# DeonDavisV/Nodexa-Chain-Core

Hardware: AMD Instinct MI355X
Metric: KawPow MH/s + Equihash(200,9) Sol/s, whole node at 1/2/4/8 MI355X (higher is better)
Workload: dtype u32; 1 GPU; model=KawPow (ProgPoW 0.9.4, RAVENCOINKAWPOW) epoch 384, 4.00 GiB DAG, height 2880123, global_batch=33553920, parallelism=dp1

## Files before the change

nodexa_chain_core_amd/hip/kernels/kawpow_anyperiod.hip:

```cpp
#include "kernel_params.h"
#include "keccak_device.hpp"

#define KA_BLOCK 256
#define KA_MIN_WAVES 6

NX_DEV uint32_t ka_fnv1a(uint32_t h, uint32_t d) { return (h ^ d) * 0x01000193u; }
NX_DEV uint32_t ka_mod(uint32_t x, const FastMod32& f) {
    const uint32_t r = x - __umulhi(x, f.mb) * f.d;
    return min(r, r - f.d);
}
NX_DEV uint32_t ka_clz(uint32_t x) { return x ? (uint32_t)__builtin_clz(x) : 32u; }

NX_DEV uint32_t ka_merge(uint32_t a, uint32_t b, uint32_t kind, uint32_t rot) {
    switch (kind) {
        case 0: return a * 33u + b;
        case 1: return (a ^ b) * 33u;
        case 2: return __builtin_rotateleft32(a, rot) ^ b;
        default: return __builtin_rotateright32(a, rot) ^ b;
    }
}

NX_DEV uint32_t ka_math(uint32_t a, uint32_t b, uint32_t kind) {
    switch (kind) {
        case 0: return a + b;
        case 1: return a * b;
        case 2: return __umulhi(a, b);
        case 3: return min(a, b);
        case 4: return __builtin_rotateleft32(a, b);
        case 5: return __builtin_rotateright32(a, b);
        case 6: return a & b;
        case 7: return a | b;
        case 8: return a ^ b;
        case 9: return ka_clz(a) + ka_clz(b);
        default: return (uint32_t)(__builtin_popcount(a) + __builtin_popcount(b));
    }
}

typedef uint32_t ka_mix_t __attribute__((ext_vector_type(32)));
NX_DEV uint32_t ka_get(const ka_mix_t& m, uint32_t i) { return m[i & 31]; }
NX_DEV void ka_set(ka_mix_t& m, uint32_t i, uint32_t v) { m[i & 31] = v; }

NX_DEV void ka_seed(const uint32_t header[8], uint64_t nonce, uint32_t st2[8]) {
    uint32_t s[25];
#pragma unroll
    for (int i = 0; i < 8; ++i) s[i] = header[i];
    s[8] = (uint32_t)nonce;
    s[9] = (uint32_t)(nonce >> 32);
    const uint32_t pad[15] = {0x72, 0x41, 0x56, 0x45, 0x4E, 0x43, 0x4F, 0x49, 0x4E, 0x4B, 0x41, 0x57, 0x50, 0x4F, 0x57};
#pragma unroll
    for (int i = 0; i < 15; ++i) s[10 + i] = pad[i];
    keccak_f800(s);
#pragma unroll
    for (int i = 0; i < 8; ++i) st2[i] = s[i];
}

NX_DEV void ka_final(const uint32_t st2[8], const uint32_t digest[8], uint32_t out[8]) {
    uint32_t s[25];
#pragma unroll
    for (int i = 0; i < 8; ++i) s[i] = st2[i];
#pragma unroll
    for (int i = 0; i < 8; ++i) s[8 + i] = digest[i];
    const uint32_t pad[9] = {0x72, 0x41, 0x56, 0x45, 0x4E, 0x43, 0x4F, 0x49, 0x4E};
#pragma unroll
    for (int i = 0; i < 9; ++i) s[16 + i] = pad[i];
    keccak_f800(s);
#pragma unroll
    for (int i = 0; i < 8; ++i) out[i] = s[i];
}

struct KaProgram {
    uint32_t w[51];
};
NX_DEV void ka_load_program(KaProgram& pg, const uint32_t* program) {
#pragma unroll
    for (int i = 0; i < 51; ++i) pg.w[i] = __builtin_amdgcn_readfirstlane(program[i]);
}

NX_DEV void ka_group_hashes(const uint4* __restrict__ dag, const FastMod32& items, const uint32_t* l1,
                            KaProgram& pg, uint32_t st0, uint32_t st1, uint32_t lane, uint32_t (&own)[8]) {
#pragma unroll 1
    for (uint32_t h = 0; h < 16; ++h) {
        ka_mix_t mix;
        {
            const uint32_t z0 = ka_fnv1a(0x811c9dc5u, __shfl(st0, (int)h, 16));
            const uint32_t w0 = ka_fnv1a(z0, __shfl(st1, (int)h, 16));
            const uint32_t jsr0 = ka_fnv1a(w0, lane);
            uint32_t kz = z0, kw = w0, kj = jsr0, kc = ka_fnv1a(jsr0, lane);
#pragma unroll
            for (int r = 0; r < 32; ++r) {
                kz = 36969u * (kz & 0xffffu) + (kz >> 16);
                kw = 18000u * (kw & 0xffffu) + (kw >> 16);
                kc = 69069u * kc + 1234567u;
                kj ^= (kj << 17);
                kj ^= (kj >> 13);
                kj ^= (kj << 5);
                mix[r] = (((kz << 16) + kw) ^ kc) + kj;
            }
        }
#pragma unroll 1
        for (uint32_t r = 0; r < 64; ++r) {
            const uint32_t index = ka_mod(__shfl(mix[0], (int)(r & 15), 16), items);
            const uint4 d = dag[(size_t)index * 16 + ((lane ^ r) & 15)];
#pragma unroll
            for (int i = 0; i < 51; ++i) asm volatile("" : "+s"(pg.w[i]));
#pragma unroll
            for (int i = 0; i < 18; ++i) {
                if (i < 11) {
                    const uint32_t op = pg.w[i];
                    const uint32_t dst = (op >> 8) & 31;
                    ka_set(mix, dst, ka_merge(ka_get(mix, dst), l1[ka_get(mix, op) & 4095u], (op >> 16) & 3, op >> 24));
                }
                const uint32_t op = pg.w[11 + i];
                const uint32_t mg = pg.w[29 + i];
                const uint32_t dst = op >> 24;
                const uint32_t v = ka_math(ka_get(mix, op), ka_get(mix, op >> 8), (op >> 16) & 15);
                ka_set(mix, dst, ka_merge(ka_get(mix, dst), v, mg & 3, mg >> 8));
            }
            const uint32_t dw[4] = {d.x, d.y, d.z, d.w};
#pragma unroll
            for (int i = 0; i < 4; ++i) {
                const uint32_t op = pg.w[47 + i];
                ka_set(mix, op, ka_merge(ka_get(mix, op), dw[i], (op >> 8) & 3, op >> 16));
            }
        }
        uint32_t lh = 0x811c9dc5u;
#pragma unroll
        for (int r = 0; r < 32; ++r) lh = ka_fnv1a(lh, mix[r]);
        const bool mine = lane == h;
#pragma unroll
        for (int k = 0; k < 8; ++k) {
            const uint32_t a = __shfl(lh, k, 16);
            const uint32_t b = __shfl(lh, k + 8, 16);
            const uint32_t word = ka_fnv1a(ka_fnv1a(0x811c9dc5u, a), b);
            own[k] = mine ? word : own[k];
        }
    }
}

extern "C" __global__ __launch_bounds__(KA_BLOCK, KA_MIN_WAVES) void kawpow_search_any(KawpowAnySearchParams p) {
    __shared__ uint32_t l1[4096];
    __shared__ uint32_t stale_word;
    if (blockDim.x != KA_BLOCK) return;
    if (threadIdx.x == 0) {
        uint32_t s = 0;
        if (p.gen_word) s = __hip_atomic_load(p.gen_word, __ATOMIC_RELAXED, __HIP_MEMORY_SCOPE_SYSTEM) != p.generation;
        stale_word = s;
        if (s) atomicAdd(&p.results->skipped, 1u);
    }
    for (int i = threadIdx.x; i < 4096; i += KA_BLOCK) l1[i] = p.l1[i];
    __syncthreads();
    if (stale_word) return;

    KaProgram pg;
    ka_load_program(pg, p.program);
    const uint32_t lane = threadIdx.x & 15;
    const uint4* dag = (const uint4*)p.dag;
#pragma unroll 1
    for (uint32_t t = threadIdx.x; t < p.granule; t += KA_BLOCK) {
        const uint64_t nonce = p.start_nonce + (uint64_t)blockIdx.x * p.granule + t;
        uint32_t st2[8], digest[8] = {0, 0, 0, 0, 0, 0, 0, 0}, fin[8];
        ka_seed(p.header, nonce, st2);
        ka_group_hashes(dag, p.items, l1, pg, st2[0], st2[1], lane, digest);
        ka_final(st2, digest, fin);
        const uint64_t head = ((uint64_t)__builtin_bswap32(fin[0]) << 32) | __builtin_bswap32(fin[1]);
        if (head <= p.target) {
            const uint32_t slot = atomicAdd(&p.results->count, 1u);
            if (slot < NODEXA_KAWPOW_MAX_SHARES) {
                KawpowShare* s = &p.results->shares[slot];
                s->nonce = nonce;
#pragma unroll
                for (int k = 0; k < 8; ++k) {
                    s->mix[k] = digest[k];
                    s->final_[k] = fin[k];
                }
            }
        }
    }
}

extern "C" __global__ __launch_bounds__(KA_BLOCK, KA_MIN_WAVES) void kawpow_hash_any(KawpowAnyHashParams p) {
    __shared__ uint32_t l1[4096];
    if (blockDim.x != KA_BLOCK) return;
    for (int i = threadIdx.x; i < 4096; i += KA_BLOCK) l1[i] = p.l1[i];
    __syncthreads();
    KaProgram pg;
    ka_load_program(pg, p.program);
    const uint32_t lane = threadIdx.x & 15;
    const uint32_t job = blockIdx.x * KA_BLOCK + threadIdx.x;
    const bool valid = job < p.num_jobs;
    const KawpowVerifyJob j = p.jobs[valid ? job : 0];
    uint32_t st2[8], digest[8] = {0, 0, 0, 0, 0, 0, 0, 0}, fin[8];
    ka_seed(j.header, j.nonce, st2);
    ka_group_hashes((const uint4*)p.dag, p.items, l1, pg, st2[0], st2[1], lane, digest);
    ka_final(st2, digest, fin);
    if (valid) {
        uint32_t* o = p.out + (size_t)job * 16;
#pragma unroll
        for (int k = 0; k < 8; ++k) {
            o[k] = digest[k];
            o[8 + k] = fin[k];
        }
    }
}
```

Before: 292.8 MH/s.

## Interleave two ProgPoW lane-hash chains per thread and compact program words

The inner ProgPoW loop now advances KA_H (default 2) independent mix states at once, so each thread issues two DAG loads per round and interleaves their dependent ALU chains to gain instruction-level parallelism. Program words are packed from 51 to 33 SGPRs, and rotate-left merges are rewritten as rotate-right so one switch case disappears. The seed Keccak is recomputed after the loop instead of keeping st2 live, which trades extra Keccak work for fewer live registers. Occupancy drops from 6 to 4 minimum waves to make room for the doubled 32-word mix arrays, which risks spilling or less latency hiding.

```diff
diff --git a/nodexa_chain_core_amd/hip/kernels/kawpow_anyperiod.hip b/nodexa_chain_core_amd/hip/kernels/kawpow_anyperiod.hip
--- a/nodexa_chain_core_amd/hip/kernels/kawpow_anyperiod.hip
+++ b/nodexa_chain_core_amd/hip/kernels/kawpow_anyperiod.hip
@@ -2,7 +2,27 @@
 #include "keccak_device.hpp"
 
 #define KA_BLOCK 256
-#define KA_MIN_WAVES 6
+#ifndef KA_H
+#define KA_H 2
+#endif
+#ifndef KA_MIN_WAVES
+#define KA_MIN_WAVES 4
+#endif
+#ifndef KA_RESEED
+#define KA_RESEED 1
+#endif
+#ifndef KA_ROTR_ONLY
+#define KA_ROTR_ONLY 1
+#endif
+#if KA_H == 1
+#define KA_EACH(X) X(0)
+#elif KA_H == 2
+#define KA_EACH(X) X(0) X(1)
+#elif KA_H == 4
+#define KA_EACH(X) X(0) X(1) X(2) X(3)
+#else
+#error "KA_H must be 1, 2 or 4"
+#endif
 
 NX_DEV uint32_t ka_fnv1a(uint32_t h, uint32_t d) { return (h ^ d) * 0x01000193u; }
 NX_DEV uint32_t ka_mod(uint32_t x, const FastMod32& f) {
@@ -11,34 +31,35 @@
 }
 NX_DEV uint32_t ka_clz(uint32_t x) { return x ? (uint32_t)__builtin_clz(x) : 32u; }
 
-NX_DEV uint32_t ka_merge(uint32_t a, uint32_t b, uint32_t kind, uint32_t rot) {
+#define KA_FOR_H _Pragma("unroll") for (int k = 0; k < KA_H; ++k)
+NX_DEV void ka_merge(uint32_t (&a)[KA_H], const uint32_t (&b)[KA_H], uint32_t kind, uint32_t rot) {
     switch (kind) {
-        case 0: return a * 33u + b;
-        case 1: return (a ^ b) * 33u;
-        case 2: return __builtin_rotateleft32(a, rot) ^ b;
-        default: return __builtin_rotateright32(a, rot) ^ b;
-    }
-}
-
-NX_DEV uint32_t ka_math(uint32_t a, uint32_t b, uint32_t kind) {
+        case 0: KA_FOR_H a[k] = a[k] * 33u + b[k]; break;
+        case 1: KA_FOR_H a[k] = (a[k] ^ b[k]) * 33u; break;
+#if !KA_ROTR_ONLY
+        case 2: KA_FOR_H a[k] = __builtin_rotateleft32(a[k], rot) ^ b[k]; break;
+#endif
+        default: KA_FOR_H a[k] = __builtin_rotateright32(a[k], rot) ^ b[k]; break;
+    }
+}
+
+NX_DEV void ka_math(uint32_t (&v)[KA_H], const uint32_t (&a)[KA_H], const uint32_t (&b)[KA_H], uint32_t kind) {
     switch (kind) {
-        case 0: return a + b;
-        case 1: return a * b;
-        case 2: return __umulhi(a, b);
-        case 3: return min(a, b);
-        case 4: return __builtin_rotateleft32(a, b);
-        case 5: return __builtin_rotateright32(a, b);
-        case 6: return a & b;
-        case 7: return a | b;
-        case 8: return a ^ b;
-        case 9: return ka_clz(a) + ka_clz(b);
-        default: return (uint32_t)(__builtin_popcount(a) + __builtin_popcount(b));
+        case 0: KA_FOR_H v[k] = a[k] + b[k]; break;
+        case 1: KA_FOR_H v[k] = a[k] * b[k]; break;
+        case 2: KA_FOR_H v[k] = __umulhi(a[k], b[k]); break;
+        case 3: KA_FOR_H v[k] = min(a[k], b[k]); break;
+        case 4: KA_FOR_H v[k] = __builtin_rotateleft32(a[k], b[k]); break;
+        case 5: KA_FOR_H v[k] = __builtin_rotateright32(a[k], b[k]); break;
+        case 6: KA_FOR_H v[k] = a[k] & b[k]; break;
+        case 7: KA_FOR_H v[k] = a[k] | b[k]; break;
+        case 8: KA_FOR_H v[k] = a[k] ^ b[k]; break;
+        case 9: KA_FOR_H v[k] = ka_clz(a[k]) + ka_clz(b[k]); break;
+        default: KA_FOR_H v[k] = (uint32_t)(__builtin_popcount(a[k]) + __builtin_popcount(b[k])); break;
     }
 }
 
 typedef uint32_t ka_mix_t __attribute__((ext_vector_type(32)));
-NX_DEV uint32_t ka_get(const ka_mix_t& m, uint32_t i) { return m[i & 31]; }
-NX_DEV void ka_set(ka_mix_t& m, uint32_t i, uint32_t v) { m[i & 31] = v; }
 
 NX_DEV void ka_seed(const uint32_t header[8], uint64_t nonce, uint32_t st2[8]) {
     uint32_t s[25];
@@ -69,70 +90,141 @@
 }
 
 struct KaProgram {
-    uint32_t w[51];
+    uint32_t w[33];
 };
+NX_DEV void ka_rotr_only(uint32_t& kind, uint32_t& rot) {
+#if KA_ROTR_ONLY
+    if (kind == 2u) {
+        kind = 3u;
+        rot = (32u - rot) & 31u;
+    }
+#endif
+}
 NX_DEV void ka_load_program(KaProgram& pg, const uint32_t* program) {
 #pragma unroll
-    for (int i = 0; i < 51; ++i) pg.w[i] = __builtin_amdgcn_readfirstlane(program[i]);
+    for (int i = 0; i < 11; ++i) {
+        const uint32_t w = __builtin_amdgcn_readfirstlane(program[i]);
+        uint32_t kind = (w >> 16) & 3u, rot = (w >> 24) & 31u;
+        ka_rotr_only(kind, rot);
+        pg.w[i] = (w & 0xffffu) | (kind << 16) | (rot << 24);
+    }
+#pragma unroll
+    for (int i = 0; i < 18; ++i) {
+        const uint32_t op = __builtin_amdgcn_readfirstlane(program[11 + i]);
+        const uint32_t mg = __builtin_amdgcn_readfirstlane(program[29 + i]);
+        uint32_t kind = mg & 3u, rot = (mg >> 8) & 31u;
+        ka_rotr_only(kind, rot);
+        pg.w[11 + i] = (op & 31u) | (((op >> 8) & 31u) << 5) | (((op >> 16) & 15u) << 10) | (((op >> 24) & 31u) << 14) |
+                       (kind << 19) | (rot << 21);
+    }
+#pragma unroll
+    for (int i = 0; i < 4; ++i) {
+        const uint32_t w = __builtin_amdgcn_readfirstlane(program[47 + i]);
+        uint32_t kind = (w >> 8) & 3u, rot = (w >> 16) & 31u;
+        ka_rotr_only(kind, rot);
+        pg.w[29 + i] = (w & 0xffu) | (kind << 8) | (rot << 16);
+    }
+}
+
+#define KA_MIX(k) m##k
+#define KA_GET(k, dstarr, idx) dstarr[k] = KA_MIX(k)[(idx) & 31];
+#define KA_SET(k, srcarr, idx) KA_MIX(k)[(idx) & 31] = srcarr[k];
+
+NX_DEV ka_mix_t ka_fill(uint32_t s0, uint32_t s1, uint32_t lane) {
+    ka_mix_t mix;
+    const uint32_t z0 = ka_fnv1a(0x811c9dc5u, s0);
+    const uint32_t w0 = ka_fnv1a(z0, s1);
+    const uint32_t jsr0 = ka_fnv1a(w0, lane);
+    uint32_t kz = z0, kw = w0, kj = jsr0, kc = ka_fnv1a(jsr0, lane);
+#pragma unroll
+    for (int r = 0; r < 32; ++r) {
+        kz = 36969u * (kz & 0xffffu) + (kz >> 16);
+        kw = 18000u * (kw & 0xffffu) + (kw >> 16);
+        kc = 69069u * kc + 1234567u;
+        kj ^= (kj << 17);
+        kj ^= (kj >> 13);
+        kj ^= (kj << 5);
+        mix[r] = (((kz << 16) + kw) ^ kc) + kj;
+    }
+    return mix;
 }
 
 NX_DEV void ka_group_hashes(const uint4* __restrict__ dag, const FastMod32& items, const uint32_t* l1,
                             KaProgram& pg, uint32_t st0, uint32_t st1, uint32_t lane, uint32_t (&own)[8]) {
 #pragma unroll 1
-    for (uint32_t h = 0; h < 16; ++h) {
-        ka_mix_t mix;
-        {
-            const uint32_t z0 = ka_fnv1a(0x811c9dc5u, __shfl(st0, (int)h, 16));
-            const uint32_t w0 = ka_fnv1a(z0, __shfl(st1, (int)h, 16));
-            const uint32_t jsr0 = ka_fnv1a(w0, lane);
-            uint32_t kz = z0, kw = w0, kj = jsr0, kc = ka_fnv1a(jsr0, lane);
-#pragma unroll
-            for (int r = 0; r < 32; ++r) {
-                kz = 36969u * (kz & 0xffffu) + (kz >> 16);
-                kw = 18000u * (kw & 0xffffu) + (kw >> 16);
-                kc = 69069u * kc + 1234567u;
-                kj ^= (kj << 17);
-                kj ^= (kj >> 13);
-                kj ^= (kj << 5);
-                mix[r] = (((kz << 16) + kw) ^ kc) + kj;
-            }
-        }
+    for (uint32_t h0 = 0; h0 < 16; h0 += KA_H) {
+#define KA_X(k) ka_mix_t KA_MIX(k) = ka_fill(__shfl(st0, (int)(h0 + k), 16), __shfl(st1, (int)(h0 + k), 16), lane);
+        KA_EACH(KA_X)
+#undef KA_X
 #pragma unroll 1
         for (uint32_t r = 0; r < 64; ++r) {
-            const uint32_t index = ka_mod(__shfl(mix[0], (int)(r & 15), 16), items);
-            const uint4 d = dag[(size_t)index * 16 + ((lane ^ r) & 15)];
-#pragma unroll
-            for (int i = 0; i < 51; ++i) asm volatile("" : "+s"(pg.w[i]));
+            uint4 d[KA_H];
+#define KA_X(k) d[k] = dag[(size_t)ka_mod(__shfl(KA_MIX(k)[0], (int)(r & 15), 16), items) * 16 + ((lane ^ r) & 15)];
+            KA_EACH(KA_X)
+#undef KA_X
+#pragma unroll
+            for (int i = 0; i < 33; ++i) asm volatile("" : "+s"(pg.w[i]));
 #pragma unroll
             for (int i = 0; i < 18; ++i) {
+                uint32_t a[KA_H], b[KA_H], v[KA_H];
                 if (i < 11) {
                     const uint32_t op = pg.w[i];
                     const uint32_t dst = (op >> 8) & 31;
-                    ka_set(mix, dst, ka_merge(ka_get(mix, dst), l1[ka_get(mix, op) & 4095u], (op >> 16) & 3, op >> 24));
+#define KA_X(k) KA_GET(k, b, op) b[k] = l1[b[k] & 4095u];
+                    KA_EACH(KA_X)
+#undef KA_X
+#define KA_X(k) KA_GET(k, a, dst)
+                    KA_EACH(KA_X)
+#undef KA_X
+                    ka_merge(a, b, (op >> 16) & 3, op >> 24);
+#define KA_X(k) KA_SET(k, a, dst)
+                    KA_EACH(KA_X)
+#undef KA_X
                 }
                 const uint32_t op = pg.w[11 + i];
-                const uint32_t mg = pg.w[29 + i];
-                const uint32_t dst = op >> 24;
-                const uint32_t v = ka_math(ka_get(mix, op), ka_get(mix, op >> 8), (op >> 16) & 15);
-                ka_set(mix, dst, ka_merge(ka_get(mix, dst), v, mg & 3, mg >> 8));
+                const uint32_t dst = op >> 14;
+#define KA_X(k) KA_GET(k, a, op)
+                KA_EACH(KA_X)
+#undef KA_X
+#define KA_X(k) KA_GET(k, b, op >> 5)
+                KA_EACH(KA_X)
+#undef KA_X
+                ka_math(v, a, b, (op >> 10) & 15);
+#define KA_X(k) KA_GET(k, a, dst)
+                KA_EACH(KA_X)
+#undef KA_X
+                ka_merge(a, v, (op >> 19) & 3, op >> 21);
+#define KA_X(k) KA_SET(k, a, dst)
+                KA_EACH(KA_X)
+#undef KA_X
             }
-            const uint32_t dw[4] = {d.x, d.y, d.z, d.w};
 #pragma unroll
             for (int i = 0; i < 4; ++i) {
-                const uint32_t op = pg.w[47 + i];
-                ka_set(mix, op, ka_merge(ka_get(mix, op), dw[i], (op >> 8) & 3, op >> 16));
+                const uint32_t op = pg.w[29 + i];
+                uint32_t a[KA_H], b[KA_H];
+#define KA_X(k) KA_GET(k, a, op) b[k] = i == 0 ? d[k].x : i == 1 ? d[k].y : i == 2 ? d[k].z : d[k].w;
+                KA_EACH(KA_X)
+#undef KA_X
+                ka_merge(a, b, (op >> 8) & 3, op >> 16);
+#define KA_X(k) KA_SET(k, a, op)
+                KA_EACH(KA_X)
+#undef KA_X
             }
         }
-        uint32_t lh = 0x811c9dc5u;
-#pragma unroll
-        for (int r = 0; r < 32; ++r) lh = ka_fnv1a(lh, mix[r]);
-        const bool mine = lane == h;
-#pragma unroll
-        for (int k = 0; k < 8; ++k) {
-            const uint32_t a = __shfl(lh, k, 16);
-            const uint32_t b = __shfl(lh, k + 8, 16);
-            const uint32_t word = ka_fnv1a(ka_fnv1a(0x811c9dc5u, a), b);
-            own[k] = mine ? word : own[k];
+        uint32_t lh[KA_H];
+#define KA_X(k) lh[k] = 0x811c9dc5u; \
+        _Pragma("unroll") for (int r = 0; r < 32; ++r) lh[k] = ka_fnv1a(lh[k], KA_MIX(k)[r]);
+        KA_EACH(KA_X)
+#undef KA_X
+        KA_FOR_H {
+            const bool mine = lane == h0 + k;
+#pragma unroll
+            for (int j = 0; j < 8; ++j) {
+                const uint32_t x = __shfl(lh[k], j, 16);
+                const uint32_t y = __shfl(lh[k], j + 8, 16);
+                const uint32_t word = ka_fnv1a(ka_fnv1a(0x811c9dc5u, x), y);
+                own[j] = mine ? word : own[j];
+            }
         }
     }
 }
@@ -157,10 +249,15 @@
     const uint4* dag = (const uint4*)p.dag;
 #pragma unroll 1
     for (uint32_t t = threadIdx.x; t < p.granule; t += KA_BLOCK) {
-        const uint64_t nonce = p.start_nonce + (uint64_t)blockIdx.x * p.granule + t;
+        uint64_t nonce = p.start_nonce + (uint64_t)blockIdx.x * p.granule + t;
         uint32_t st2[8], digest[8] = {0, 0, 0, 0, 0, 0, 0, 0}, fin[8];
         ka_seed(p.header, nonce, st2);
         ka_group_hashes(dag, p.items, l1, pg, st2[0], st2[1], lane, digest);
+#if KA_RESEED
+        nonce = p.start_nonce + (uint64_t)blockIdx.x * p.granule + t;
+        asm volatile("" : "+v"(nonce));
+        ka_seed(p.header, nonce, st2);
+#endif
         ka_final(st2, digest, fin);
         const uint64_t head = ((uint64_t)__builtin_bswap32(fin[0]) << 32) | __builtin_bswap32(fin[1]);
         if (head <= p.target) {
```

After: 292.2 MH/s. No clear change (-0.2%).
